# MKLab-ITI/multimedia-indexing

Hardware: AMD Instinct MI355X
Metric: queries/sec @ recall@1, IVFPQ 100Mx128-d nprobe=32 (higher is better)
Workload: dtype f64; 1 GPU; IVFPQ 100000000x128-d, 8192 coarse cells, nprobe w=32, m=16x256, k=100, batch 16384 queries/step; n=100000000, dim=128, cells=8192, nprobe=32, m=16, ks=256, k=100, batch=16384, batch_per_gpu=16384

## Files before the change

### multimedia-indexing_amd/csrc/mmidx_api.hip

```cpp
#include "../../include/mmidx.h"
#include "mmidx_kernels.h"
#include "mmidx_scan_grp.h"
#include "mmidx_scan_mfma.h"
#include "mmidx_scan_mfma_kc.h"
#include "mmidx_scan_mfma_a.h"
#include "mmidx_scan_q.h"
#include "mmidx_host.h"

#include <algorithm>
#include <cmath>
#include <condition_variable>
#include <cstdarg>
#include <cstdio>
#include <cstring>
#include <deque>
#include <functional>
#include <mutex>
#include <string>
#include <limits>
#include <vector>

namespace {

thread_local std::string g_err;
// ... 914 lines not shown
    return 4 * nq >= 5 * std::max<int64_t>(1, h->nonempty_lists) && h->n_csr / std::max<int64_t>(1, h->nonempty_lists) >= 4096;
}

template <int M, int DSUB>
int launch_q_t(const QParams &QP, unsigned grid, size_t lds, hipStream_t st) {
    static int static_lds = -1;
    if (static_lds < 0) {
        hipFuncAttributes fa{};
        HIPCK(hipFuncGetAttributes(&fa, (const void *)k_scan_q<M, DSUB>));
        static_lds = (int)fa.sharedSizeBytes;
    }
    if (static_lds != 0) return mmidx_fail(MMIDX_ERR_UNSUPPORTED, "k_scan_q owns %d bytes of static LDS: its table is not at LDS address 0", static_lds);
    HIPCK(hipFuncSetAttribute((const void *)k_scan_q<M, DSUB>, hipFuncAttributeMaxDynamicSharedMemorySize, (int)lds));
    hipLaunchKernelGGL((k_scan_q<M, DSUB>), dim3(grid), dim3(256), lds, st, QP);
    HIPCK(hipGetLastError());
    return MMIDX_OK;
}

int launch_passa_q(mmidx_index *h, const ScanParams &P, const SearchPlan &pl, long long nq, hipStream_t st) {
    constexpr int G = MMIDX_Q_G;
    const int C = h->C;
    const size_t nfb = (size_t)nq * (size_t)std::max(pl.nchunks, 1);
    HIPCK(h->ws_pcount.reserve((size_t)C + 1));
    HIPCK(h->ws_pstart.reserve((size_t)C + 1));
    HIPCK(h->ws_pcursor.reserve((size_t)C));
    HIPCK(h->ws_order.reserve((size_t)nq * (size_t)P.w));
    const size_t max_groups = (size_t)nq / G + (size_t)std::min<long long>(nq, C) + 8;
    HIPCK(h->ws_gdesc.reserve(max_groups));
    HIPCK(h->ws_gfb.reserve(8));
    if (h->ws_fb.cap < 2 * nfb + 4) {
        HIPCK(h->ws_fb.reserve(2 * nfb + 4));
        HIPCK(hipMemsetAsync(h->ws_fb.p, 0, 4 * sizeof(int32_t), st));
    }
    const unsigned gq = (unsigned)((nq + 255) / 256);
    hipLaunchKernelGGL(k_a1_pair_count, dim3(gq), dim3(256), 0, st, P.cells, P.w, (long long)nq, P.list_off, h->ws_pcount.p, C);
    hipLaunchKernelGGL(k_q_scan_groups, dim3(1), dim3(1024), 0, st, h->ws_pcount.p, C, G, h->ws_pstart.p, h->ws_pcursor.p, h->ws_gdesc.p, h->ws_gfb.p);
    hipLaunchKernelGGL(k_a1_pair_scatter, dim3(gq), dim3(256), 0, st, P.cells, P.w, (long long)nq, P.list_off, h->ws_pstart.p, h->ws_pcursor.p, h->ws_order.p);
    HIPCK(hipGetLastError());
    QParams QP{};
    QP.S = P;
    QP.S.order = h->ws_order.p;
    QP.S.n_order = h->ws_pstart.p + C;
    QP.S.rot = h->d_rot;
    QP.S.perm = h->d_perm;
    QP.S.fb_count = (u32 *)h->ws_fb.p;
    QP.S.fb_items = h->ws_fb.p + 4;
    QP.S.fb_ch = h->ws_fb.p + 4 + nfb;
    QP.gdesc = h->ws_gdesc.p;
    QP.n_groups = h->ws_gfb.p;
    QP.pq = h->d_pq;
    QP.pqstat = h->d_pqstat;
    QP.pqT32 = h->d_pqT32;
    QP.pmax = h->rmax;
    QP.timing = nullptr;
    const QLds L(h->m, h->D);
    const unsigned grid = (unsigned)((std::min<size_t>(max_groups, (size_t)nq) + 7 + 7) & ~(size_t)7);
    int rc;
    switch (h->dsub) {
        case 4: rc = launch_q_t<16, 4>(QP, grid, L.total, st); break;
        case 8: rc = launch_q_t<16, 8>(QP, grid, L.total, st); break;
        default: rc = launch_q_t<16, 16>(QP, grid, L.total, st); break;
    }
    if (rc) return rc;
    if (h->sw.debug_sync) {
        int32_t c4[4], ng = 0;
        (void)hipStreamSynchronize(st);
        (void)hipMemcpy(c4, h->ws_fb.p, sizeof(c4), hipMemcpyDeviceToHost);
        (void)hipMemcpy(&ng, h->ws_gfb.p, sizeof(ng), hipMemcpyDeviceToHost);
        fprintf(stderr, "[mmidx] K3q: %lld queries in %d groups (grid %u, lds %zu); %d (query, chunk) items handed back to K3\n", nq, ng, grid, L.total, c4[0]);
    }
    ScanParams F = P;
    F.cap = pl.cap;
    F.fb_count = QP.S.fb_count;
    F.fb_items = QP.S.fb_items;
    F.fb_ch = QP.S.fb_ch;
    F.order = QP.S.fb_items;
    F.n_order = (const int32_t *)QP.S.fb_count;
    F.order_ch = P.ivf ? QP.S.fb_ch : nullptr;
    F.n_items = (int)nfb;
    return launch_scan(h, F, dim3((unsigned)nfb, 1), pl.lds, st);
}

struct PassaMfmaShape {
    int sub, nsub;
    size_t max_groups, bm_stride;
    bool fits;
};
PassaMfmaShape passa_mfma_shape(const mmidx_index *h, long long npairs) {
    constexpr int G = MF_QG;
    PassaMfmaShape S{};
    const long long maxlen = std::max<long long>(h->max_list_len, 1);
    int sub = h->sw.mfma_sub;
    if (sub <= 0) {
        const long long est_groups = npairs / G + std::min<long long>(npairs, std::max<int64_t>(1, h->nonempty_lists));
        const long long want = 4ll * 2 * std::max(h->num_cus, 8);
        long long pieces = std::max<long long>(1, std::min<long long>(8, (want + est_groups - 1) / est_groups));
        long long sb = (maxlen + pieces - 1) / pieces;
        sb = std::max<long long>(1024, sb);
        sub = (int)((sb + 63) & ~63ll);
    }
    sub = (std::max(sub, 64) + 31) & ~31;
    if ((maxlen + sub - 1) / sub > 8) sub = (int)((((maxlen + 7) / 8) + 31) & ~31ll);
    S.sub = sub;
    S.nsub = (int)((maxlen + sub - 1) / sub);
    S.max_groups = (size_t)npairs / G + (size_t)std::min<long long>(npairs, h->C) + 1;
    S.bm_stride = (size_t)((sub + 31) / 32) * 256;
// ... 1258 lines not shown
            rc = launch_scan_grouped(h, P, pl, (long long)nq, npairs, st);
            if (rc == 1) {
                const unsigned gx = (unsigned)(((P.n_items + 7) / 8) * 8);
                rc = launch_scan_filtered(h, P, pl, dim3(gx, (unsigned)pl.nchunks), st);
            }
            if (rc) return rc;
            DBG_SYNC("pass B scan");
        }
        if (prof) HIPCK(hipEventRecord(ev[3], st));
        if (prof) h->launches += (two_pass ? 1 : 0) + (phase != 2 ? 1 : 0);
    } else {
        if (plight) {
            HIPCK(hipEventRecord(ev[2], st));
            HIPCK(hipEventRecord(ev[5], st));
        }
        if (prof) {
            HIPCK(hipEventRecord(ev[2], st));
            HIPCK(hipEventRecord(ev[5], st));
            HIPCK(hipEventRecord(ev[3], st));
        }
        if (phase == 1) {
            hipLaunchKernelGGL(k_T_export, dim3((unsigned)((nq + 255) / 256)), dim3(256), 0, st, h->ws_T.p, d_T_io, (long long)nq);
            HIPCK(hipGetLastError());
            if (prof) HIPCK(hipEventRecord(ev[4], st));
            return MMIDX_OK;
        }
    }
    MergeParams M{};
    M.T = h->ws_T.p;
    M.pool_cnt = h->ws_pcnt.p;
    M.pool_key = h->ws_pkey.p;
    M.pool_val = h->ws_pval.p;
    M.poolq = pl.poolq;
    M.cells = ivf ? d_cells : nullptr;
    M.list_off = h->d_off;
    M.ids = h->d_ids;
    M.w = P.w;
    M.k = k;
    M.mode = mode;
    M.iid_out = d_iid;
    M.dist_out = d_dist;
    M.count_out = d_cnt;
    M.flag_out = h->ws_flag.p;
    M.pdist = d_pdist;
    M.pkey = d_pkey;
    if (mode == 1 && phase == 2 && h->shard_dest) {
        M.dest = h->shard_dest;
        M.dest_per = h->shard_dest_per;
        M.dest_me = h->shard_dest_me;
    }
    int mcap = 512;
    while (mcap < 2 * pl.K1) mcap <<= 1;
    M.cap = mcap;
    const size_t mlds = (size_t)mcap * 16 + ((ivf && P.w <= 1024) ? (size_t)P.w * 8 : 0);
    if (pl.K1 <= 128) {
        HIPCK(hipFuncSetAttribute((const void *)k_merge<128>, hipFuncAttributeMaxDynamicSharedMemorySize, (int)mlds));
        hipLaunchKernelGGL(k_merge<128>, dim3((unsigned)nq), dim3(128), mlds, st, M);
    } else {
        HIPCK(hipFuncSetAttribute((const void *)k_merge<MMIDX_BLOCK>, hipFuncAttributeMaxDynamicSharedMemorySize, (int)mlds));
        hipLaunchKernelGGL(k_merge<MMIDX_BLOCK>, dim3((unsigned)nq), dim3(MMIDX_BLOCK), mlds, st, M);
    }
    HIPCK(hipGetLastError());
    DBG_SYNC("merge");
    if (mode == 0 && h->n_csr > 0) {
        TieParams TP{};
        TP.S = P;
        TP.flag = h->ws_flag.p;
        TP.ids = h->d_ids;
        TP.iid_out = d_iid;
        TP.dist_out = d_dist;
        TP.k = k;
        TP.nq = (int)nq;
        const unsigned tgrid = (unsigned)std::min<int64_t>((nq + MMIDX_BLOCK - 1) / MMIDX_BLOCK, 4096);
        const size_t tlds = (P.glut ? 0 : (size_t)h->m * h->ks * 8) + 2 * (size_t)h->D * 8;
        if (P.glut) {
            if ((size_t)nq > h->glut_slots) return mmidx_fail(MMIDX_ERR_UNSUPPORTED, "lookup-table scratch too small for the tie replay");
            if (sdc_tt) {
                hipLaunchKernelGGL((k_tie_resolve<unsigned char, true, true>), dim3(tgrid), dim3(MMIDX_BLOCK), tlds, st, TP);
            } else if (h->code_bytes == 1) {
                hipLaunchKernelGGL((k_tie_resolve<unsigned char, false, true>), dim3(tgrid), dim3(MMIDX_BLOCK), tlds, st, TP);
            } else {
                hipLaunchKernelGGL((k_tie_resolve<unsigned short, false, true>), dim3(tgrid), dim3(MMIDX_BLOCK), tlds, st, TP);
            }
        } else if (sdc_tt) {
            HIPCK(hipFuncSetAttribute((const void *)k_tie_resolve<unsigned char, true>, hipFuncAttributeMaxDynamicSharedMemorySize, (int)tlds));
            hipLaunchKernelGGL((k_tie_resolve<unsigned char, true>), dim3(tgrid), dim3(MMIDX_BLOCK), tlds, st, TP);
        } else if (h->code_bytes == 1) {
            HIPCK(hipFuncSetAttribute((const void *)k_tie_resolve<unsigned char, false>, hipFuncAttributeMaxDynamicSharedMemorySize, (int)tlds));
            hipLaunchKernelGGL((k_tie_resolve<unsigned char, false>), dim3(tgrid), dim3(MMIDX_BLOCK), tlds, st, TP);
        } else {
            HIPCK(hipFuncSetAttribute((const void *)k_tie_resolve<unsigned short, false>, hipFuncAttributeMaxDynamicSharedMemorySize, (int)tlds));
            hipLaunchKernelGGL((k_tie_resolve<unsigned short, false>), dim3(tgrid), dim3(MMIDX_BLOCK), tlds, st, TP);
        }
        HIPCK(hipGetLastError());
    }
    if (prof) {
        HIPCK(hipEventRecord(ev[4], st));
        if (!ivf) h->host_codes += nq * h->n_csr;
        if (ivf || mode == 0) {
            const long long tot = (long long)nq * h->w;
            hipLaunchKernelGGL(k_count_stats, dim3(256), dim3(256), 0, st, ivf ? d_cells : nullptr, h->d_off, tot, h->w,
                               mode == 0 ? h->ws_flag.p : nullptr, (long long)nq, h->d_counters);
        }
        HIPCK(hipGetLastError());
    }
    return MMIDX_OK;
}
// ... 1535 lines not shown
```

### multimedia-indexing_amd/csrc/mmidx_kernels.h

```cpp
#pragma once
#include <hip/hip_runtime.h>
#include <stdint.h>

#include "mmidx_device_util.h"
#include "mmidx_host.h"

#define MMIDX_BLOCK 256
#define MMIDX_KEY_MAX 0xFFFFFFFFFFFFFFFFull

__device__ __forceinline__ u64 dkey(double d) { return (u64)__double_as_longlong(d); }
__device__ __forceinline__ double keyd(u64 k) { return __longlong_as_double((long long)k); }

template <typename V>
__device__ __forceinline__ void block_bitonic_sort(u64 *key, V *val, int n) {
    for (int size = 2; size <= n; size <<= 1) {
        for (int stride = size >> 1; stride > 0; stride >>= 1) {
            __syncthreads();
            for (int t = threadIdx.x; t < (n >> 1); t += blockDim.x) {
                int lo = 2 * t - (t & (stride - 1));
                int hi = lo + stride;
                bool up = ((lo & size) == 0);
                u64 ka = key[lo], kb = key[hi];
                V va = val[lo], vb = val[hi];
                bool gt = (ka > kb) || (ka == kb && va > vb);
                if (gt == up) {
                    key[lo] = kb;
                    key[hi] = ka;
                    val[lo] = vb;
                    val[hi] = va;
                }
            }
        }
    }
    __syncthreads();
}

__device__ __forceinline__ u32 wave_min_u32(u32 x) {
    u32 v = x;
#define MMIDX_DPP_MIN(ctrl, rmask)                                                              \
    {                                                                                           \
        const u32 o = (u32)__builtin_amdgcn_update_dpp((int)v, (int)v, ctrl, rmask, 0xf, false); \
        v = o < v ? o : v;                                                                      \
    }
    MMIDX_DPP_MIN(0x111, 0xf) MMIDX_DPP_MIN(0x112, 0xf) MMIDX_DPP_MIN(0x114, 0xf) MMIDX_DPP_MIN(0x118, 0xf)
    MMIDX_DPP_MIN(0x142, 0xa) MMIDX_DPP_MIN(0x143, 0xc)
#undef MMIDX_DPP_MIN
    return wave_read_u32(v, 63);
}
__device__ __forceinline__ u32 wave_max_u32(u32 x) { return ~wave_min_u32(~x); }
__device__ __forceinline__ double wave_read_f64(double x, int l) {
    const u64 b = (u64)__double_as_longlong(x);
    const u32 lo_ = wave_read_u32((u32)b, l), hi_ = wave_read_u32((u32)(b >> 32), l);
    return __longlong_as_double((long long)(((u64)hi_ << 32) | lo_));
}

__device__ __forceinline__ int pow2ceil(int n) {
    int p = 1;
    while (p < n) p <<= 1;
// ... 3335 lines not shown
        run += (u32)cnt[c];
    }
    if (tid == 1023) {
        start[C] = (int32_t)(base + incl);
        if (host_hint) *host_hint = (int32_t)(base + incl);
    }
}
__global__ void k_pair_scatter(const int32_t *__restrict__ cells, int w, int rank_lo, long long npairs,
                               const int32_t *__restrict__ start, int32_t *__restrict__ cursor,
                               int32_t *__restrict__ order, const unsigned char *__restrict__ keep) {
    const long long e = (long long)blockIdx.x * blockDim.x + threadIdx.x;
    if (e >= npairs) return;
    if ((int)(e % w) < rank_lo) return;
    if (!keep[e]) return;
    const int c = cells[e];
    const int pos = start[c] + atomicAdd(cursor + c, 1);
    order[pos] = (int32_t)e;
}

#define MMIDX_MCAP 2048
#define MMIDX_K_MAX 4095
struct ShardDest {
    double *pd;
    long long *pk;
    int32_t *pc;
};
struct MergeParams {
    const u64 *T;
    const u32 *pool_cnt;
    const u64 *pool_key;
    const u64 *pool_val;
    int poolq;
    const int32_t *cells;
    const int64_t *list_off;
    const int32_t *ids;
    int w, k, mode;
    int cap;
    int32_t *iid_out;
    double *dist_out;
    int32_t *count_out;
    int32_t *flag_out;
    double *pdist;
    long long *pkey;
    const ShardDest *dest;
    int dest_per, dest_me;
};

template <int NT>
__global__ __launch_bounds__(NT) void k_merge(const MergeParams P) {
    extern __shared__ __attribute__((aligned(16))) unsigned char smem[];
    const int CAP = P.cap;
    u64 *key = (u64 *)smem;
    u64 *val = key + CAP;
    int64_t *s_off = (int64_t *)(val + CAP);
    const int q = blockIdx.x, tid = threadIdx.x;
    const int K1 = P.k + 1;
    __shared__ u32 s_m;
    int n = (int)P.pool_cnt[q];
    if (n > P.poolq) n = P.poolq;
    const u64 *pk = P.pool_key + (size_t)q * P.poolq;
    const u64 *pv = P.pool_val + (size_t)q * P.poolq;
    double *o_pd = P.pdist;
    long long *o_pk = P.pkey;
    int32_t *o_pc = P.count_out + q;
    if (P.mode == 1) {
        size_t row = (size_t)q * K1;
        if (P.dest) {
            const int o = q / P.dest_per, ql = q - o * P.dest_per;
            const ShardDest d = P.dest[o];
            row = ((size_t)P.dest_me * P.dest_per + ql) * K1;
            o_pd = d.pd;
            o_pk = d.pk;
            o_pc = d.pc + (size_t)P.dest_me * P.dest_per + ql;
        }
        o_pd += row;
        o_pk += row;
    }
    if (n == 0 && P.mode == 1) {
        if (tid == 0) *o_pc = 0;
        return;
    }
    const u64 T = P.T ? __hip_atomic_load(P.T + q, __ATOMIC_RELAXED, __HIP_MEMORY_SCOPE_AGENT) : MMIDX_KEY_MAX;
    if (tid == 0) s_m = 0;
    const bool offs_in_lds = P.cells && P.w <= 1024;
    if (offs_in_lds)
        for (int t = tid; t < P.w; t += NT) s_off[t] = P.list_off[P.cells[(size_t)q * P.w + t]];
    auto list_start = [&](int rank) -> int64_t {
        if (offs_in_lds) return s_off[rank];
        return P.list_off[P.cells ? P.cells[(size_t)q * P.w + rank] : 0];
    };
    __syncthreads();
    {
        const u64 lane_lt = (1ull << (tid & 63)) - 1ull;
        for (int base0 = 0; base0 < n; base0 += NT) {
            const int e = base0 + tid;
            u64 kk = MMIDX_KEY_MAX, vv = 0;
            if (e < n) {
                kk = pk[e];
                vv = pv[e];
            }
            const bool pass = e < n && kk <= T;
            const u64 mask = __ballot(pass);
            if (mask) {
                u32 base = 0;
                const int leader = __ffsll((long long)mask) - 1;
                if ((tid & 63) == leader) base = atomicAdd(&s_m, (u32)__popcll(mask));
                base = wave_read_u32(base, leader);
                if (pass) {
                    const u32 slot = base + (u32)__popcll(mask & lane_lt);
                    if (slot < (u32)CAP) {
                        key[slot] = kk;
                        val[slot] = vv;
                    }
                }
            }
        }
    }
    __syncthreads();
    const int m = (int)s_m;
    int kept = 0;
    if (m <= NT) {
        const bool have = tid < m;
        const u64 mk = have ? key[tid] : MMIDX_KEY_MAX, mv = have ? val[tid] : MMIDX_KEY_MAX;
        int rank = 0, eqc = 0;
        for (int j = 0; j < m; j++) {
            const u64 ok = key[j];
            rank += ok < mk;
            eqc += ok == mk;
        }
        if (__builtin_amdgcn_ballot_w64(have && eqc > 1)) {
            rank = 0;
            for (int j = 0; j < m; j++) {
                const u64 ok = key[j], ov = val[j];
                rank += (ok < mk) || (ok == mk && ov < mv);
            }
        }
        __syncthreads();
        if (have) {
            key[rank] = mk;
            val[rank] = mv;
        }
        __syncthreads();
        kept = m < K1 ? m : K1;
    } else if (m <= CAP) {
        const int Pn = pow2ceil(m);
        for (int i = m + tid; i < Pn; i += NT) {
            key[i] = MMIDX_KEY_MAX;
            val[i] = MMIDX_KEY_MAX;
        }
        block_bitonic_sort<u64>(key, val, Pn);
        kept = m < K1 ? m : K1;
    } else {
        int consumed = 0;
        do {
            int take = n - consumed;
            if (take > CAP - kept) take = CAP - kept;
            __syncthreads();
            for (int i = tid; i < take; i += NT) {
                key[kept + i] = pk[consumed + i];
                val[kept + i] = pv[consumed + i];
            }
            const int filled = kept + take;
            const int Pn = pow2ceil(filled < 2 ? 2 : filled);
            for (int i = filled + tid; i < Pn; i += NT) {
                key[i] = MMIDX_KEY_MAX;
                val[i] = MMIDX_KEY_MAX;
            }
            block_bitonic_sort<u64>(key, val, Pn);
            consumed += take;
            kept = filled < K1 ? filled : K1;
        } while (consumed < n);
    }
    const int total = kept;
    const int cnt = total < P.k ? total : P.k;
    if (P.mode == 1) {
        const int nwrite = P.dest ? total : K1;
        for (int i = tid; i < nwrite; i += NT) {
            double dd = __longlong_as_double(0x7FF0000000000000ll);
            long long kk = -1;
            if (i < total) {
                const u64 v = val[i];
                const int rank = (int)(v >> 32);
                const u32 pos = (u32)v;
                const int iid = P.ids[list_start(rank) + pos];
                dd = keyd(key[i]);
                kk = (long long)(((u64)rank << 32) | (u32)iid);
            }
            o_pd[i] = dd;
            o_pk[i] = kk;
        }
        if (tid == 0) *o_pc = total;
        return;
    }
    for (int i = tid; i < P.k; i += NT) {
        int iid = -1;
        double dd = __longlong_as_double(0x7FF0000000000000ll);
        if (i < cnt) {
            int a = i, b = i;
            const u64 ki = key[i];
            while (a > 0 && key[a - 1] == ki) a--;
            while (b + 1 < cnt && key[b + 1] == ki) b++;
            const int src = a + (b - i);
            const u64 v = val[src];
            const int rank = (int)(v >> 32);
            const u32 pos = (u32)v;
            iid = P.ids[list_start(rank) + pos];
            dd = keyd(ki);
        }
        P.iid_out[(size_t)q * P.k + i] = iid;
        P.dist_out[(size_t)q * P.k + i] = dd;
    }
    if (tid == 0) {
        P.count_out[q] = cnt;
        P.flag_out[q] = (total > P.k && key[P.k - 1] == key[P.k]) ? 1 : 0;
    }
}

template <int NT>
__global__ __launch_bounds__(NT) void k_merge_partials(int k, int nq, int nshards, int mcap,
                                                       const double *__restrict__ pdist,
                                                       const long long *__restrict__ pkey,
                                                       const int32_t *__restrict__ pcount,
                                                       const long long *__restrict__ poff,
                                                       int32_t *iid_out, double *dist_out,
                                                       int32_t *count_out, int32_t *flag_out, int32_t *nflag_out) {
    extern __shared__ __attribute__((aligned(16))) unsigned char smem[];
    u64 *key = (u64 *)smem;
    u64 *val = key + mcap;
    const int q = blockIdx.x, tid = threadIdx.x;
    const int K1 = k + 1;
    int kept = 0;
    for (int s = 0; s < nshards;) {
        int filled = kept;
        while (s < nshards) {
            int c = pcount[(size_t)s * nq + q];
            if (c > K1) c = K1;
            if (filled + c > mcap) break;
            const size_t base = poff ? (size_t)poff[(size_t)s * nq + q] : ((size_t)s * nq + q) * K1;
            for (int i = tid; i < c; i += NT) {
                key[filled + i] = dkey(pdist[base + i]);
                val[filled + i] = (u64)pkey[base + i];
            }
            filled += c;
            s++;
        }
        if (kept == 0 && s == nshards && filled <= NT) {
            __syncthreads();
            const bool have = tid < filled;
            const u64 mk = have ? key[tid] : MMIDX_KEY_MAX, mv = have ? val[tid] : MMIDX_KEY_MAX;
            int rank = 0, eqc = 0;
            for (int j = 0; j < filled; j++) {
                const u64 ok = key[j];
                rank += ok < mk;
                eqc += ok == mk;
            }
            if (__builtin_amdgcn_ballot_w64(have && eqc > 1)) {
                rank = 0;
                for (int j = 0; j < filled; j++) {
                    const u64 ok = key[j], ov = val[j];
// ... 893 lines not shown
```

### multimedia-indexing_amd/csrc/mmidx_scan_q.h

```cpp
#pragma once
#include <type_traits>
#ifndef Q_STOP
#define Q_STOP 0
#endif

#define MMIDX_Q_G 4
#define MMIDX_Q_SLOTS 6
#define MMIDX_Q_HKQ 192
#ifndef MMIDX_Q_U
#define MMIDX_Q_U 8
#endif
#define MMIDX_Q_SCALE 4000.0
#ifndef Q_STAGSEL
#define Q_STAGSEL (blockIdx.x >> 8)
#endif
#ifndef Q_WPS
#define Q_WPS 4
#endif
#ifndef Q_TU
#define Q_TU 4
#endif
#ifndef Q_CH
#define Q_CH 4
#endif
#ifndef Q_FR
#define Q_FR 2
#endif

struct QParams {
    ScanParams S;
    const int4 *gdesc;
    const int32_t *n_groups;
    const double *pq;
    const double *pqstat;
    const float *pqT32;
    double pmax;
    unsigned long long *timing;
};

typedef unsigned int q_u32x2 __attribute__((ext_vector_type(2)));
typedef __attribute__((address_space(3))) const q_u32x2 lds_cuint2;
typedef __attribute__((address_space(3))) const unsigned int lds_cu32;

struct QLds {
    size_t tab, res, misc, cent, sel, total;
    __host__ __device__ QLds(int M, int D) {
        size_t o = 0;
        tab = o; o += (size_t)M * 2048;
        res = o; o += (size_t)MMIDX_Q_G * D * 8;
        misc = o; o += 64 * 8;
        cent = o;
        {
            const size_t a = (size_t)MMIDX_Q_G * MMIDX_Q_HKQ * 4, b = (size_t)D * 16;
            o += a > b ? a : b;
        }
        sel = tab;
        total = (o + 15) & ~(size_t)15;
    }
};

__device__ __forceinline__ u32 q_med3(u32 a, u32 b, u32 c) {
    u32 r;
    asm("v_med3_u32 %0, %1, %2, %3" : "=v"(r) : "v"(a), "v"(b), "v"(c));
    return r;
}
typedef float q_f2 __attribute__((ext_vector_type(2)));
typedef float q_f4 __attribute__((ext_vector_type(4)));
typedef double q_d2 __attribute__((ext_vector_type(2)));
__device__ __forceinline__ q_f2 q_pk_sub_lo(q_f2 r, q_f2 p) {
    q_f2 d;
    asm("v_pk_add_f32 %0, %1, %2 op_sel:[0,0] op_sel_hi:[1,0] neg_lo:[0,1] neg_hi:[0,1]" : "=v"(d) : "v"(r), "v"(p));
    return d;
}
__device__ __forceinline__ q_f2 q_pk_sub_hi(q_f2 r, q_f2 p) {
    q_f2 d;
    asm("v_pk_add_f32 %0, %1, %2 op_sel:[0,1] op_sel_hi:[1,1] neg_lo:[0,1] neg_hi:[0,1]" : "=v"(d) : "v"(r), "v"(p));
    return d;
}
__device__ __forceinline__ q_f2 q_pk_fma(q_f2 a, q_f2 b, q_f2 c) {
    q_f2 d;
    asm("v_pk_fma_f32 %0, %1, %2, %3" : "=v"(d) : "v"(a), "v"(b), "v"(c));
    return d;
}
__device__ __forceinline__ q_f2 q_pk_mul(q_f2 a, q_f2 b) {
    q_f2 d;
    asm("v_pk_mul_f32 %0, %1, %2" : "=v"(d) : "v"(a), "v"(b));
    return d;
}
template <int SH>
// ... 75 lines not shown
            cnt[c] = 0;
            emit(c, n);
        }
    }
    if (tid == 1023) {
        cnt[C] = 0;
        start[C] = (int32_t)(ba + ia);
        *n_groups = (int32_t)(bb + ib);
    }
}

#ifdef Q_TIMING
#define Q_T(n) do { if (tid == 0) { const unsigned long long t_ = __builtin_readcyclecounter(); atomicAdd(QP.timing + (n), t_ - qt_last); qt_last = t_; } } while (0)
#else
#define Q_T(n) do {} while (0)
#endif
template <int M, int DSUB, int GA>
__device__ __forceinline__ void q_scan_group(const QParams &QP, const int4 gd, unsigned char *smem) {
    constexpr int G = MMIDX_Q_G, NT = 256, WV = 4, U = MMIDX_Q_U, HKQ = MMIDX_Q_HKQ, NS = MMIDX_Q_SLOTS;
    static_assert(G == WV, "wave i takes query i in the selection");
    static_assert(M * 2048 >= G * MMIDX_Q_HKQ * 8, "the candidates' exact sums re-use the table");
    static_assert(M <= 16 && M * 4095 < 65535, "K3q's 16-bit sums hold at most sixteen saturated entries");
    const ScanParams &P = QP.S;
    const int D = P.D;
    const QLds L(M, D);
    double *s_r = (double *)(smem + L.res);
    int *s_astar = (int *)(smem + L.misc);
    u32 *s_flag = (u32 *)(smem + L.misc) + 4;
    u32 *s_kept = (u32 *)(smem + L.misc) + 8;
    u32 *s_emit = (u32 *)(smem + L.misc) + 12;
    u32 *s_base = (u32 *)(smem + L.misc) + 16;
    double *s_inv = (double *)(smem + L.misc) + 16;
    u64 *s_max = (u64 *)(smem + L.misc) + 20;
    u32 *s_cut = (u32 *)(smem + L.misc) + 24;
    u32 *cent = (u32 *)(smem + L.cent);

    const int cell = gd.x, ng = gd.z;
    const int tid = threadIdx.x, lane = tid & 63, wv = tid >> 6;
#ifdef Q_TIMING
    unsigned long long qt_last = __builtin_readcyclecounter();
#endif
    int qid[G];
#pragma unroll
    for (int i = 0; i < G; i++) qid[i] = P.order[gd.y + (i < ng ? i : 0)] / P.w;
    const int64_t beg = P.list_off[cell];
    const u32 n_seg = (u32)__builtin_amdgcn_readfirstlane((int)(u32)(P.list_off[cell + 1] - beg));
    if (n_seg == 0) return;
    const unsigned char *codes0;
    {
        const u64 e0 = (u64)beg;
        const u32 lo32 = (u32)__builtin_amdgcn_readfirstlane((int)(u32)e0), hi32 = (u32)__builtin_amdgcn_readfirstlane((int)(u32)(e0 >> 32));
        codes0 = (const unsigned char *)P.codes + (size_t)(((u64)hi32 << 32) | lo32) * M;
    }
    auto fetch = [&](CodeVec<M, unsigned char> &dst, const u32 i) {
        const u32 ic = min(i, n_seg - 1u);
        dst.load(codes0 + ic * (u32)M);
    };
    CodeVec<M, unsigned char> X0[U], X1[U];
#pragma unroll
    for (int u = 0; u < U; u++) fetch(X0[u], (u32)u * NT + (u32)tid);

    static_assert(M % Q_TU == 0, "the table is built Q_TU rows at a time");
    static_assert(DSUB % 2 == 0, "two dimensions per load");
    auto load_rows = [&](q_f2 (&p)[Q_TU][DSUB / 2], const int s0) {
#pragma unroll
        for (int j = 0; j < Q_TU; j++)
#pragma unroll
            for (int t2 = 0; t2 < DSUB / 2; t2++) p[j][t2] = ((const q_f2 *)QP.pqT32)[((size_t)(s0 + j) * (DSUB / 2) + t2) * 256 + tid];
    };
    float *r32 = (float *)(smem + L.cent);

    for (int i = tid; i < 128; i += NT) ((u32 *)(smem + L.misc))[i] = 0;
    __syncthreads();
    if (wv < GA) {
        const int i = wv;
        const double *qrow = P.Q + (size_t)qid[i] * D, *crow = P.coarse + (size_t)cell * D;
        if (P.transform == 1) {
            double *raw = (double *)smem + (size_t)i * D;
            for (int d = lane; d < D; d += 64) raw[d] = crow[d] - qrow[d];
            __builtin_amdgcn_s_waitcnt(0);
            __builtin_amdgcn_wave_barrier();
            for (int j = lane; j < D; j += 64) {
                double total = 0.0;
                for (int k = 0; k < D; k++) total += raw[k] * P.rot[(size_t)k * D + j];
                s_r[(size_t)i * D + j] = total;
            }
        } else {
            for (int d = lane; d < D; d += 64) {
                const int src = P.transform == 2 ? P.perm[d] : d;
                s_r[(size_t)i * D + d] = crow[src] - qrow[src];
            }
        }
        __builtin_amdgcn_s_waitcnt(0);
        __builtin_amdgcn_wave_barrier();
        double part = 0.0, rr = 0.0;
        for (int d = lane; d < D; d += 64) {
            const double r = s_r[(size_t)i * D + d];
            part += r * r - 2.0 * r * QP.pqstat[d];
            rr += r * r;
            r32[d * 4 + i] = (float)r;
        }
        if (lane < M) part += QP.pqstat[M * DSUB + lane];
        const double qr = wave_sum_f64(part);
        const double rnx = sqrt(wave_sum_f64(rr)) + QP.pmax;
        const bool fits = qr > 1e-24 && qr < 1e24 && rnx < 1e15 && 2.0 * 5.9604644775390625e-8 * sqrt(4128.0 * (MMIDX_Q_SCALE / qr)) * rnx <= 0.25;
        const bool ok = i < ng && fits;
// ... 202 lines not shown
#pragma unroll
        for (int k = 0; k < NS; k++) {
            const u32 key = slot[i][k];
            if (key != 0xFFFFFFFFu && (key >> 16) <= cut) push(i, key >> 16, ((key & 0xFFFFu) << 8) | (u32)tid);
        }
        const u32 last = slot[i][NS - 1];
        if (last != 0xFFFFFFFFu && (last >> 16) <= cut) rmask |= 1u << i;
    }
    if (rmask) *s_resc = 1u;
    __syncthreads();
    if (*s_resc) {
        build_table(std::false_type{});
        __syncthreads();
        if (rmask) {
#pragma unroll
            for (int i = 0; i < GA; i++) {
                if (!((rmask >> i) & 1u)) continue;
                const u32 cut = s_cut[i], last = slot[i][NS - 1];
                for (u32 step = 0; step * NT + (u32)tid < n_seg; step++) {
                    CodeVec<M, unsigned char> cv;
                    cv.load(codes0 + (step * NT + (u32)tid) * (u32)M);
                    u32 lo, hi;
                    lookup(cv, lo, hi);
                    const u32 a = (i & 1) ? ((i < 2 ? lo : hi) >> 16) : ((i < 2 ? lo : hi) & 0xFFFFu);
                    if (a <= cut && ((a << 16) | step) > last) push(i, a, (step << 8) | (u32)tid);
                }
            }
        }
    }
    __syncthreads();
    Q_T(3);
    bool live[G];
    u32 first[G + 1];
    first[0] = 0;
#pragma unroll
    for (int i = 0; i < G; i++) {
        live[i] = i < ng && s_flag[i] == 0u && s_kept[i] <= (u32)HKQ;
        if (i < ng && !live[i] && tid == 0) {
            const u32 nch = (n_seg + (u32)P.chunk - 1u) / (u32)P.chunk;
            const u32 sl = atomicAdd(P.fb_count, nch);
            for (u32 c = 0; c < nch; c++) {
                P.fb_items[sl + c] = qid[i] * P.w;
                P.fb_ch[sl + c] = (int32_t)c;
            }
        }
        first[i + 1] = first[i] + (live[i] ? s_kept[i] : 0u);
    }
    const u32 ncand = first[G];
    if (ncand == 0) return;
    u64 *ckey = (u64 *)smem;
    constexpr int RB = DSUB * 8, LPR = RB / 16, RPL = LPR ? 64 / LPR : 0, MB = CodeVec<M, unsigned char>::WORDS * 4;
    constexpr size_t XC = (size_t)G * HKQ * 8, XT = XC + (size_t)NT * MB;
    constexpr bool COOP = RB % 16 == 0 && LPR >= 1 && 16 % LPR == 0 && XT + (size_t)WV * 64 * RB <= (size_t)M * 2048;
    auto which = [&](const u32 idx) -> int {
        int i = 0;
#pragma unroll
        for (int k = 1; k < G; k++) i += (idx >= first[k]) ? 1 : 0;
        return i;
    };
    auto entry_of = [&](const u32 idx, const int i) -> u32 { return cent[i * HKQ + (idx - (i == 0 ? first[0] : (i == 1 ? first[1] : (i == 2 ? first[2] : first[3]))))]; };
    if constexpr (COOP) {
        unsigned char *s_code = smem + XC + (size_t)wv * 64 * MB;
        unsigned char *s_tile = smem + XT + (size_t)wv * 64 * RB;
        const u32 row0 = (u32)lane / LPR, chunk = (u32)lane % LPR;
        auto sums = [&](const u32 idx) {
            const bool h = idx < ncand;
            if (!__builtin_amdgcn_ballot_w64(h)) return;
            const u32 ic = h ? idx : ncand - 1u;
            const int q = which(ic);
            const u32 v = entry_of(ic, q);
            {
                CodeVec<M, unsigned char> cv;
                cv.load(codes0 + (v & 0xFFFFFFu) * (u32)M);
#pragma unroll
                for (int i = 0; i < MB / 4; i++) ((u32 *)(s_code + (size_t)lane * MB))[i] = cv.wd[i];
            }
            __builtin_amdgcn_wave_barrier();
            const q_d2 *tq = (const q_d2 *)(s_r + (size_t)q * D);
            double d = 0.0;
            const u32 rot0 = (row0 / (16 / LPR)) % LPR, rotl = ((u32)lane / (16 / LPR)) % LPR;
            const u32 srcoff = ((chunk + rot0) % LPR) * 16u;
            auto bytes = [&](u32 (&b)[LPR], const int s) {
#pragma unroll
                for (int i = 0; i < LPR; i++) b[i] = s_code[((u32)i * RPL + row0) * MB + (u32)s];
            };
            auto dma = [&](const u32 (&b)[LPR], const int s) {
#pragma unroll
                for (int i = 0; i < LPR; i++)
                    __builtin_amdgcn_global_load_lds((const __attribute__((address_space(1))) void *)((const char *)QP.pq + (((u32)s * 256u + b[i]) * (u32)RB + srcoff)),
                                                     (__attribute__((address_space(3))) void *)(s_tile + i * 1024), 16, 0, 0);
            };
            u32 cb[LPR];
            bytes(cb, 0);
            dma(cb, 0);
#pragma unroll 1
            for (int s = 0; s < M; s++) {
                q_d2 p2[LPR];
                bytes(cb, s + 1 < M ? s + 1 : s);
                __builtin_amdgcn_s_waitcnt(0x0F70);
#pragma unroll
                for (int c = 0; c < LPR; c++) p2[c] = *(const q_d2 *)(s_tile + (u32)lane * RB + (((u32)c - rotl) % LPR) * 16u);
                __builtin_amdgcn_s_waitcnt(0xC07F);
                if (s + 1 < M) dma(cb, s + 1);
                double a = 0.0;
#pragma unroll
                for (int c = 0; c < LPR; c++) {
                    const q_d2 r = tq[s * LPR + c];
                    const double f0 = r.x - p2[c].x, f1 = r.y - p2[c].y;
                    a += f0 * f0;
                    a += f1 * f1;
                }
                d = s == 0 ? a : d + a;
            }
            if (h) {
                ckey[idx] = dkey(d);
                if (v & 0x80000000u) atomicMax(s_max + q, dkey(d));
            }
        };
        sums((u32)tid);
        sums((u32)tid + NT);
        sums((u32)tid + 2 * NT);
    } else {
        const u32 ia = (u32)tid, ib = (u32)tid + NT, ic = (u32)tid + 2 * NT;
        auto sum2 = [&](const u32 i0, const u32 i1) {
            const bool h0 = i0 < ncand, h1 = i1 < ncand;
            if (!__builtin_amdgcn_ballot_w64(h0)) return;
            const int q0 = h0 ? which(i0) : 0, q1 = h1 ? which(i1) : 0;
            const u32 v0 = h0 ? entry_of(i0, q0) : 0u, v1 = h1 ? entry_of(i1, q1) : 0u;
            CodeVec<M, unsigned char> c0v, c1v;
            c0v.load(codes0 + (v0 & 0xFFFFFFu) * (u32)M);
            c1v.load(codes0 + (v1 & 0xFFFFFFu) * (u32)M);
            const double *t0 = s_r + (size_t)q0 * D, *t1 = s_r + (size_t)q1 * D;
            double d0 = 0.0, d1 = 0.0;
#pragma unroll 1
            for (int s0 = 0; s0 < M; s0 += Q_FR) {
                double p0[Q_FR][DSUB], p1[Q_FR][DSUB];
#pragma unroll
                for (int j = 0; j < Q_FR; j++) {
                    const u32 b0 = (c0v.wd[(s0 + j) >> 2] >> (8 * ((s0 + j) & 3))) & 0xffu, b1 = (c1v.wd[(s0 + j) >> 2] >> (8 * ((s0 + j) & 3))) & 0xffu;
                    const double *r0 = QP.pq + ((size_t)(s0 + j) * 256 + (size_t)b0) * DSUB;
                    const double *r1 = QP.pq + ((size_t)(s0 + j) * 256 + (size_t)b1) * DSUB;
#pragma unroll
                    for (int t = 0; t < DSUB; t++) {
                        p0[j][t] = r0[t];
                        p1[j][t] = r1[t];
                    }
                }
#pragma unroll
                for (int j = 0; j < Q_FR; j++) {
                    double a0 = 0.0, a1 = 0.0;
#pragma unroll
                    for (int t = 0; t < DSUB; t++) {
                        const double f0 = t0[(s0 + j) * DSUB + t] - p0[j][t], f1 = t1[(s0 + j) * DSUB + t] - p1[j][t];
                        a0 += f0 * f0;
                        a1 += f1 * f1;
                    }
                    d0 = (s0 + j) == 0 ? a0 : d0 + a0;
                    d1 = (s0 + j) == 0 ? a1 : d1 + a1;
                }
            }
            if (h0) {
                ckey[i0] = dkey(d0);
                if (v0 & 0x80000000u) atomicMax(s_max + q0, dkey(d0));
            }
            if (h1) {
                ckey[i1] = dkey(d1);
                if (v1 & 0x80000000u) atomicMax(s_max + q1, dkey(d1));
            }
        };
        sum2(ia, 0xFFFFFFFFu);
        sum2(ib, 0xFFFFFFFFu);
        sum2(ic, 0xFFFFFFFFu);
    }
    __syncthreads();
    Q_T(4);
    u64 Te[G];
#pragma unroll
    for (int i = 0; i < G; i++) {
        const bool has_T = live[i] && s_astar[i] >= 0;
        const u64 Tl = has_T ? s_max[i] : MMIDX_KEY_MAX;
        const u64 Tg = __hip_atomic_load(P.T + qid[i], __ATOMIC_RELAXED, __HIP_MEMORY_SCOPE_AGENT);
        Te[i] = Tl < Tg ? Tl : Tg;
        if (has_T && tid == 0) atomicMin(P.T + qid[i], Tl);
    }
#pragma unroll 1
    for (u32 idx = (u32)tid; idx < ncand; idx += NT) {
        int i = 0;
#pragma unroll
        for (int k = 1; k < G; k++) i += (idx >= first[k]) ? 1 : 0;
        const u64 te = i == 0 ? Te[0] : (i == 1 ? Te[1] : (i == 2 ? Te[2] : Te[3]));
        u32 *ce = cent + i * HKQ + (idx - (i == 0 ? first[0] : (i == 1 ? first[1] : (i == 2 ? first[2] : first[3]))));
        const u32 v = *ce & 0xFFFFFFu;
        const u32 sl = ckey[idx] <= te ? atomicAdd(s_emit + i, 1u) : 0xFFu;
        *ce = v | (sl << 24);
    }
    __syncthreads();
    if (tid < G && s_emit[tid]) s_base[tid] = atomicAdd(P.pool_cnt + qid[tid], s_emit[tid]);
    __syncthreads();
#pragma unroll 1
    for (u32 idx = (u32)tid; idx < ncand; idx += NT) {
        int i = 0;
#pragma unroll
        for (int k = 1; k < G; k++) i += (idx >= first[k]) ? 1 : 0;
        const u32 v = cent[i * HKQ + (idx - (i == 0 ? first[0] : (i == 1 ? first[1] : (i == 2 ? first[2] : first[3]))))];
        if ((v >> 24) == 0xFFu) continue;
        const int qq = i == 0 ? qid[0] : (i == 1 ? qid[1] : (i == 2 ? qid[2] : qid[3]));
        const u32 sl = s_base[i] + (v >> 24);
        if (sl < (u32)P.poolq) {
            P.pool_key[(size_t)qq * P.poolq + sl] = ckey[idx];
            P.pool_val[(size_t)qq * P.poolq + sl] = (u64)(v & 0xFFFFFFu);
        }
    }
    Q_T(5);
}

template <int M, int DSUB>
__global__ __launch_bounds__(256, Q_WPS) void k_scan_q(const QParams QP) {
    extern __shared__ __attribute__((aligned(16))) unsigned char smem[];
    const int grp = (int)blockIdx.x;
    if (grp >= *QP.n_groups) return;
    const int4 gd = QP.gdesc[grp];
#ifndef Q_NO_GA2
    if (gd.z <= 2) q_scan_group<M, DSUB, 2>(QP, gd, smem);
    else
#endif
        q_scan_group<M, DSUB, 4>(QP, gd, smem);
}
```

Measured before the change: 21.58 million queries/s.

## Carry candidate ids through the pool and prefetch pool entries in merge

The query-grouped scan kernel now fetches each candidate's global id into LDS with asynchronous global-to-LDS loads while it computes distances. It packs that id into the pool value, so the merge kernel can skip the dependent list_off/cells/ids lookup chain when every entry carries an id and no more than one block's worth survives. The merge kernel also issues its first pool load before reading the count and batches several loads per thread. The risk is a 24-bit position limit and extra ids traffic in the scan for candidates that are later rejected.

```diff
diff --git a/multimedia-indexing_amd/csrc/mmidx_api.hip b/multimedia-indexing_amd/csrc/mmidx_api.hip
--- a/multimedia-indexing_amd/csrc/mmidx_api.hip
+++ b/multimedia-indexing_amd/csrc/mmidx_api.hip
@@ -990,6 +990,7 @@
     QP.pqstat = h->d_pqstat;
     QP.pqT32 = h->d_pqT32;
     QP.pmax = h->rmax;
+    QP.ids = h->d_ids;
     QP.timing = nullptr;
     const QLds L(h->m, h->D);
     const unsigned grid = (unsigned)((std::min<size_t>(max_groups, (size_t)nq) + 7 + 7) & ~(size_t)7);
@@ -2354,7 +2355,7 @@
     int mcap = 512;
     while (mcap < 2 * pl.K1) mcap <<= 1;
     M.cap = mcap;
-    const size_t mlds = (size_t)mcap * 16 + ((ivf && P.w <= 1024) ? (size_t)P.w * 8 : 0);
+    const size_t mlds = (size_t)mcap * 16 + (size_t)(pl.K1 <= 128 ? 128 : MMIDX_BLOCK) * 4 + ((ivf && P.w <= 1024) ? (size_t)P.w * 8 : 0);
     if (pl.K1 <= 128) {
         HIPCK(hipFuncSetAttribute((const void *)k_merge<128>, hipFuncAttributeMaxDynamicSharedMemorySize, (int)mlds));
         hipLaunchKernelGGL(k_merge<128>, dim3((unsigned)nq), dim3(128), mlds, st, M);
diff --git a/multimedia-indexing_amd/csrc/mmidx_kernels.h b/multimedia-indexing_amd/csrc/mmidx_kernels.h
--- a/multimedia-indexing_amd/csrc/mmidx_kernels.h
+++ b/multimedia-indexing_amd/csrc/mmidx_kernels.h
@@ -4,6 +4,7 @@
 
 #include "mmidx_device_util.h"
 #include "mmidx_host.h"
+#include "mmidx_pool_entry.h"
 
 #define MMIDX_BLOCK 256
 #define MMIDX_KEY_MAX 0xFFFFFFFFFFFFFFFFull
@@ -3445,14 +3446,27 @@
     const int CAP = P.cap;
     u64 *key = (u64 *)smem;
     u64 *val = key + CAP;
-    int64_t *s_off = (int64_t *)(val + CAP);
+    u32 *cid = (u32 *)(val + CAP);
+    int64_t *s_off = (int64_t *)(cid + NT);
     const int q = blockIdx.x, tid = threadIdx.x;
     const int K1 = P.k + 1;
-    __shared__ u32 s_m;
-    int n = (int)P.pool_cnt[q];
-    if (n > P.poolq) n = P.poolq;
+    __shared__ u32 s_m, s_lack;
     const u64 *pk = P.pool_key + (size_t)q * P.poolq;
     const u64 *pv = P.pool_val + (size_t)q * P.poolq;
+    constexpr int PF = 4;
+    u64 ck[PF], cv[PF];
+    const bool spec = P.mode == 0;
+    const int e0 = (spec && tid < P.poolq) ? tid : 0;
+    ck[0] = pk[e0];
+    cv[0] = pv[e0];
+    int n = (int)P.pool_cnt[q];
+    const u64 T = P.T ? __hip_atomic_load(P.T + q, __ATOMIC_RELAXED, __HIP_MEMORY_SCOPE_AGENT) : MMIDX_KEY_MAX;
+#pragma unroll
+    for (int c = 1; c < PF; c++) {
+        ck[c] = MMIDX_KEY_MAX;
+        cv[c] = 0;
+    }
+    if (n > P.poolq) n = P.poolq;
     double *o_pd = P.pdist;
     long long *o_pk = P.pkey;
     int32_t *o_pc = P.count_out + q;
@@ -3473,48 +3487,72 @@
         if (tid == 0) *o_pc = 0;
         return;
     }
-    const u64 T = P.T ? __hip_atomic_load(P.T + q, __ATOMIC_RELAXED, __HIP_MEMORY_SCOPE_AGENT) : MMIDX_KEY_MAX;
-    if (tid == 0) s_m = 0;
-    const bool offs_in_lds = P.cells && P.w <= 1024;
-    if (offs_in_lds)
-        for (int t = tid; t < P.w; t += NT) s_off[t] = P.list_off[P.cells[(size_t)q * P.w + t]];
+    if (tid == 0) {
+        s_m = 0;
+        s_lack = 0;
+    }
+    __syncthreads();
+    {
+        const u64 lane_lt = (1ull << (tid & 63)) - 1ull;
+        bool lack = false;
+        auto compact = [&](const int e, const u64 kk, const u64 vv) {
+            const bool pass = e < n && kk <= T;
+            const u64 mask = __ballot(pass);
+            if (!mask) return;
+            u32 base = 0;
+            const int leader = __ffsll((long long)mask) - 1;
+            if ((tid & 63) == leader) base = atomicAdd(&s_m, (u32)__popcll(mask));
+            base = wave_read_u32(base, leader);
+            if (pass) {
+                const u32 slot = base + (u32)__popcll(mask & lane_lt);
+                if (slot < (u32)CAP) {
+                    key[slot] = kk;
+                    val[slot] = pool_val_ord(vv);
+                }
+                if (slot < (u32)NT) cid[slot] = (u32)pool_val_iid(vv);
+                lack |= !pool_val_has_id(vv);
+            }
+        };
+        for (int base0 = 0; base0 < n; base0 += PF * NT) {
+#pragma unroll
+            for (int c = 0; c < PF; c++) {
+                const int e = base0 + c * NT + tid;
+                if (e < n && !(spec && base0 == 0 && c == 0)) {
+                    ck[c] = pk[e];
+                    cv[c] = pv[e];
+                }
+            }
+#pragma unroll
+            for (int c = 0; c < PF; c++)
+                if (base0 + c * NT < n) compact(base0 + c * NT + tid, ck[c], cv[c]);
+        }
+        if (lack) s_lack = 1u;
+    }
+    __syncthreads();
+    const int m = (int)s_m;
+    const bool lookup = s_lack != 0u || m > NT;
+    const bool offs_in_lds = lookup && P.cells && P.w <= 1024;
+    int64_t off_t = 0;
+    if (offs_in_lds && tid < P.w) off_t = P.list_off[P.cells[(size_t)q * P.w + tid]];
+    auto store_offs = [&]() {
+        if (!offs_in_lds) return;
+        if (tid < P.w) s_off[tid] = off_t;
+        for (int t = tid + NT; t < P.w; t += NT) s_off[t] = P.list_off[P.cells[(size_t)q * P.w + t]];
+    };
     auto list_start = [&](int rank) -> int64_t {
         if (offs_in_lds) return s_off[rank];
         return P.list_off[P.cells ? P.cells[(size_t)q * P.w + rank] : 0];
     };
-    __syncthreads();
-    {
-        const u64 lane_lt = (1ull << (tid & 63)) - 1ull;
-        for (int base0 = 0; base0 < n; base0 += NT) {
-            const int e = base0 + tid;
-            u64 kk = MMIDX_KEY_MAX, vv = 0;
-            if (e < n) {
-                kk = pk[e];
-                vv = pv[e];
-            }
-            const bool pass = e < n && kk <= T;
-            const u64 mask = __ballot(pass);
-            if (mask) {
-                u32 base = 0;
-                const int leader = __ffsll((long long)mask) - 1;
-                if ((tid & 63) == leader) base = atomicAdd(&s_m, (u32)__popcll(mask));
-                base = wave_read_u32(base, leader);
-                if (pass) {
-                    const u32 slot = base + (u32)__popcll(mask & lane_lt);
-                    if (slot < (u32)CAP) {
-                        key[slot] = kk;
-                        val[slot] = vv;
-                    }
-                }
-            }
-        }
-    }
-    __syncthreads();
-    const int m = (int)s_m;
+    auto id_of = [&](const int i) -> int {
+        if (!lookup) return (int)cid[i];
+        const u64 v = val[i];
+        return P.ids[list_start((int)(v >> 32)) + (u32)v];
+    };
     int kept = 0;
     if (m <= NT) {
         const bool have = tid < m;
         const u64 mk = have ? key[tid] : MMIDX_KEY_MAX, mv = have ? val[tid] : MMIDX_KEY_MAX;
+        const u32 mi = have ? cid[tid] : 0u;
         int rank = 0, eqc = 0;
         for (int j = 0; j < m; j++) {
             const u64 ok = key[j];
@@ -3528,14 +3566,17 @@
                 rank += (ok < mk) || (ok == mk && ov < mv);
             }
         }
+        store_offs();
         __syncthreads();
         if (have) {
             key[rank] = mk;
             val[rank] = mv;
+            cid[rank] = mi;
         }
         __syncthreads();
         kept = m < K1 ? m : K1;
     } else if (m <= CAP) {
+        store_offs();
         const int Pn = pow2ceil(m);
         for (int i = m + tid; i < Pn; i += NT) {
             key[i] = MMIDX_KEY_MAX;
@@ -3544,6 +3585,7 @@
         block_bitonic_sort<u64>(key, val, Pn);
         kept = m < K1 ? m : K1;
     } else {
+        store_offs();
         int consumed = 0;
         do {
             int take = n - consumed;
@@ -3551,7 +3593,7 @@
             __syncthreads();
             for (int i = tid; i < take; i += NT) {
                 key[kept + i] = pk[consumed + i];
-                val[kept + i] = pv[consumed + i];
+                val[kept + i] = pool_val_ord(pv[consumed + i]);
             }
             const int filled = kept + take;
             const int Pn = pow2ceil(filled < 2 ? 2 : filled);
@@ -3572,10 +3614,8 @@
             double dd = __longlong_as_double(0x7FF0000000000000ll);
             long long kk = -1;
             if (i < total) {
-                const u64 v = val[i];
-                const int rank = (int)(v >> 32);
-                const u32 pos = (u32)v;
-                const int iid = P.ids[list_start(rank) + pos];
+                const int rank = (int)(val[i] >> 32);
+                const int iid = id_of(i);
                 dd = keyd(key[i]);
                 kk = (long long)(((u64)rank << 32) | (u32)iid);
             }
@@ -3593,11 +3633,7 @@
             const u64 ki = key[i];
             while (a > 0 && key[a - 1] == ki) a--;
             while (b + 1 < cnt && key[b + 1] == ki) b++;
-            const int src = a + (b - i);
-            const u64 v = val[src];
-            const int rank = (int)(v >> 32);
-            const u32 pos = (u32)v;
-            iid = P.ids[list_start(rank) + pos];
+            iid = id_of(a + (b - i));
             dd = keyd(ki);
         }
         P.iid_out[(size_t)q * P.k + i] = iid;
diff --git a/multimedia-indexing_amd/csrc/mmidx_pool_entry.h b/multimedia-indexing_amd/csrc/mmidx_pool_entry.h
--- /dev/null
+++ b/multimedia-indexing_amd/csrc/mmidx_pool_entry.h
@@ -0,0 +1,18 @@
+#pragma once
+#include <stdint.h>
+
+#if defined(__HIPCC__) || defined(__CUDACC__)
+#define MMIDX_PE_FN __host__ __device__ __forceinline__
+#else
+#define MMIDX_PE_FN static inline
+#endif
+
+#define MMIDX_PE_POS_BITS 24
+
+MMIDX_PE_FN uint64_t pool_val_legacy(uint32_t probe_rank, uint32_t pos) { return ((uint64_t)probe_rank << 32) | (uint64_t)pos; }
+MMIDX_PE_FN uint64_t pool_val_carried(int32_t iid, uint32_t pos) {
+    return (1ull << 63) | ((uint64_t)(uint32_t)iid << MMIDX_PE_POS_BITS) | (uint64_t)(pos & ((1u << MMIDX_PE_POS_BITS) - 1u));
+}
+MMIDX_PE_FN bool pool_val_has_id(uint64_t v) { return (v >> 63) != 0; }
+MMIDX_PE_FN uint64_t pool_val_ord(uint64_t v) { return pool_val_has_id(v) ? (v & ((1ull << MMIDX_PE_POS_BITS) - 1ull)) : v; }
+MMIDX_PE_FN int32_t pool_val_iid(uint64_t v) { return (int32_t)(uint32_t)(v >> MMIDX_PE_POS_BITS); }
diff --git a/multimedia-indexing_amd/csrc/mmidx_scan_q.h b/multimedia-indexing_amd/csrc/mmidx_scan_q.h
--- a/multimedia-indexing_amd/csrc/mmidx_scan_q.h
+++ b/multimedia-indexing_amd/csrc/mmidx_scan_q.h
@@ -35,6 +35,7 @@
     const double *pqstat;
     const float *pqT32;
     double pmax;
+    const int32_t *ids;
     unsigned long long *timing;
 };
 
@@ -216,6 +217,7 @@
         const u32 lo32 = (u32)__builtin_amdgcn_readfirstlane((int)(u32)e0), hi32 = (u32)__builtin_amdgcn_readfirstlane((int)(u32)(e0 >> 32));
         codes0 = (const unsigned char *)P.codes + (size_t)(((u64)hi32 << 32) | lo32) * M;
     }
+    const int32_t *ids0 = QP.ids + (size_t)(((u64)(u32)__builtin_amdgcn_readfirstlane((int)(u32)((u64)beg >> 32)) << 32) | (u32)__builtin_amdgcn_readfirstlane((int)(u32)(u64)beg));
     auto fetch = [&](CodeVec<M, unsigned char> &dst, const u32 i) {
         const u32 ic = min(i, n_seg - 1u);
         dst.load(codes0 + ic * (u32)M);
@@ -524,6 +526,13 @@
     constexpr int RB = DSUB * 8, LPR = RB / 16, RPL = LPR ? 64 / LPR : 0, MB = CodeVec<M, unsigned char>::WORDS * 4;
     constexpr size_t XC = (size_t)G * HKQ * 8, XT = XC + (size_t)NT * MB;
     constexpr bool COOP = RB % 16 == 0 && LPR >= 1 && 16 % LPR == 0 && XT + (size_t)WV * 64 * RB <= (size_t)M * 2048;
+    constexpr size_t XI = COOP ? XT + (size_t)WV * 64 * RB : XC;
+    static_assert(XI + (size_t)G * HKQ * 4 <= (size_t)M * 2048, "the candidates' ids re-use the table");
+    u32 *cid = (u32 *)(smem + XI);
+    auto ask_id = [&](const u32 idx, const u32 pos) {
+        __builtin_amdgcn_global_load_lds((const __attribute__((address_space(1))) void *)(ids0 + pos),
+                                         (__attribute__((address_space(3))) void *)(cid + (idx - (u32)lane)), 4, 0, 0);
+    };
     auto which = [&](const u32 idx) -> int {
         int i = 0;
 #pragma unroll
@@ -569,11 +578,13 @@
             for (int s = 0; s < M; s++) {
                 q_d2 p2[LPR];
                 bytes(cb, s + 1 < M ? s + 1 : s);
-                __builtin_amdgcn_s_waitcnt(0x0F70);
+                if (s == 1) __builtin_amdgcn_s_waitcnt(0x0F71);
+                else __builtin_amdgcn_s_waitcnt(0x0F70);
 #pragma unroll
                 for (int c = 0; c < LPR; c++) p2[c] = *(const q_d2 *)(s_tile + (u32)lane * RB + (((u32)c - rotl) % LPR) * 16u);
                 __builtin_amdgcn_s_waitcnt(0xC07F);
                 if (s + 1 < M) dma(cb, s + 1);
+                if (s == 0) ask_id(idx, v & 0xFFFFFFu);
                 double a = 0.0;
 #pragma unroll
                 for (int c = 0; c < LPR; c++) {
@@ -602,6 +613,8 @@
             CodeVec<M, unsigned char> c0v, c1v;
             c0v.load(codes0 + (v0 & 0xFFFFFFu) * (u32)M);
             c1v.load(codes0 + (v1 & 0xFFFFFFu) * (u32)M);
+            ask_id(i0, v0 & 0xFFFFFFu);
+            if (__builtin_amdgcn_ballot_w64(h1)) ask_id(i1, v1 & 0xFFFFFFu);
             const double *t0 = s_r + (size_t)q0 * D, *t1 = s_r + (size_t)q1 * D;
             double d0 = 0.0, d1 = 0.0;
 #pragma unroll 1
@@ -644,6 +657,7 @@
         sum2(ib, 0xFFFFFFFFu);
         sum2(ic, 0xFFFFFFFFu);
     }
+    __builtin_amdgcn_s_waitcnt(0x0F70);
     __syncthreads();
     Q_T(4);
     u64 Te[G];
@@ -680,7 +694,7 @@
         const u32 sl = s_base[i] + (v >> 24);
         if (sl < (u32)P.poolq) {
             P.pool_key[(size_t)qq * P.poolq + sl] = ckey[idx];
-            P.pool_val[(size_t)qq * P.poolq + sl] = (u64)(v & 0xFFFFFFu);
+            P.pool_val[(size_t)qq * P.poolq + sl] = pool_val_carried((int32_t)cid[idx], v & 0xFFFFFFu);
         }
     }
     Q_T(5);
```

Result: slower. 21.35 million queries/s (-1.1%).
